# hanmekim/SceneLib2

Measured on NVIDIA H100. Metric: EKF-SLAM frames/sec @320x240 N=100 feats, higher is better.
Workload: dtype f64 (EKF, scores) + u8/int32 (correlation sums)

## Files before the change

### scenelib2_b200/csrc/search.cu

```cuda
#include "sl2_common.cuh"
#include "sl2_ptx.cuh"
#include "sl2_score.cuh"

namespace {

__device__ __forceinline__ void tma_load_3d(uint32_t dst, const CUtensorMap *map, uint32_t bar,
                                            int c0, int c1, int c2) {
  asm volatile(
      "cp.async.bulk.tensor.3d.shared::cluster.global.mbarrier::complete_tx::bytes "
      "[%0], [%1, {%3, %4, %5}], [%2];" ::"r"(dst),
      "l"(map), "r"(bar), "r"(c0), "r"(c1), "r"(c2)
      : "memory");
}

struct SearchLayout {
  int tcw, tch;
  int list, bar, vtab, per_warp;
};
__host__ __device__ inline SearchLayout search_layout(int tile_w, int tile_h, int box) {
  SearchLayout l;
  l.tcw = tile_w - 15 - box + 1;
  l.tch = tile_h - box + 1;
  const int tile_bytes = ((tile_w * tile_h + 16 + 127) / 128) * 128;
  const int max_tasks = l.tcw * ((l.tch + SL2_STRIP - 1) / SL2_STRIP);
  const int list_bytes = ((max_tasks * 4 + 15) / 16) * 16;
  const int col_bytes = ((l.tcw * 4 + 15) / 16) * 16;
  const int vtab_bytes = l.tch * 16 > col_bytes ? l.tch * 16 : col_bytes;
  l.list = tile_bytes;
  l.bar = tile_bytes + list_bytes;
  l.vtab = l.bar + 16;
  l.per_warp = ((l.vtab + vtab_bytes + 127) / 128) * 128;
  return l;
}

struct DumpPtrs {
  double *corr;
  double *sd;
  uint8_t *inside;
  int *box;
  int cap;
};

template <int BOX, bool FILTER>
__global__ void __launch_bounds__(SL2_SEARCH_WARPS * 32, FILTER ? (BOX <= 11 ? 4 : 3) : 2)
    search_kernel(const __grid_constant__ CUtensorMap tmap, const Sl2Dev d, const SearchLaunch L,
                  const DumpPtrs dump) {
  constexpr int NW = (BOX + 3) / 4;
  constexpr int HALF = (BOX - 1) / 2;
  constexpr int V = SL2_STRIP;
  constexpr uint32_t LASTMASK = (BOX % 4 == 0) ? 0xffffffffu : ((1u << (8 * (BOX % 4))) - 1u);
  extern __shared__ __align__(128) uint8_t smem[];
  pdl_prologue();

  const int warp = threadIdx.x >> 5, lane = threadIdx.x & 31;
  const int groups = (L.jobs_per_stream + SL2_SEARCH_WARPS - 1) / SL2_SEARCH_WARPS;
  const int sl = blockIdx.x / groups;
  const int r = (blockIdx.x % groups) * SL2_SEARCH_WARPS + warp;
  if (r >= L.jobs_per_stream) return;
  const int job = sl * L.jobs_per_stream + r;
  const int feat = L.job_feat[job];
  if (feat < 0) return;
  const int s = L.stream_lo + sl;

  const int TW = d.tile_w, TH = d.tile_h;
  const SearchLayout lay = search_layout(TW, TH, BOX);
  const int TCW = lay.tcw, TCH = lay.tch;
  uint8_t *tile = smem + (size_t)warp * lay.per_warp;
  uint32_t *list = reinterpret_cast<uint32_t *>(tile + lay.list);
  const uint32_t bar = smem_u32(tile + lay.bar);
  double2 *vtab = reinterpret_cast<double2 *>(tile + lay.vtab);
  short2 *colrange = reinterpret_cast<short2 *>(vtab);
  const uint32_t tile_s = smem_u32(tile);

  if (lane == 0) {
    mbar_init(bar, 1);
    fence_barrier_init();
    fence_proxy_async();
  }
  __syncwarp();

  uint32_t T[BOX][NW];
  {
    const uint32_t *pp =
        reinterpret_cast<const uint32_t *>(d.patches + ((size_t)s * d.Nmax + feat) * (BOX * 16));
#pragma unroll
    for (int rr = 0; rr < BOX; ++rr)
#pragma unroll
      for (int k = 0; k < NW; ++k) T[rr][k] = __ldg(pp + rr * 4 + k);
  }
  int Sg0 = 0, Sg0sq = 0;
#pragma unroll
  for (int rr = 0; rr < BOX; ++rr)
#pragma unroll
    for (int k = 0; k < NW; ++k) {
      Sg0 = __dp4a(T[rr][k], 0x01010101u, (uint32_t)Sg0);
      Sg0sq = __dp4a(T[rr][k], T[rr][k], (uint32_t)Sg0sq);
    }
  const PatchConst pconst = patch_const(BOX, Sg0, Sg0sq);
  const double V0d = fma(pconst.n, (double)Sg0sq, -((double)Sg0 * (double)Sg0));
  const float V0f = (float)V0d;
  const bool patch_ok = !(pconst.sigmag0 < 10.0);
  float bmin = 3.0e38f;

  const double P00 = L.job_puinv[job * 3 + 0], P01 = L.job_puinv[job * 3 + 1],
               P11 = L.job_puinv[job * 3 + 2];
  const double cx = L.job_centre[job * 2 + 0], cy = L.job_centre[job * 2 + 1];
  const int uc = __double2int_rz(add_(cx, 0.5));
  const int vc = __double2int_rz(add_(cy, 0.5));
  const SearchBox sb = search_box(P00, P01, P11, uc, vc, stream_width(d.cams[s]), stream_height(d.cams[s]), HALF);
  const Ellipse ell = make_ellipse(P00, P01, P11);
  const int CW = sb.cols(), CH = sb.rows();
  const int x0 = uc + sb.us - HALF, y0 = vc + sb.vs - HALF;
  if (!FILTER && lane == 0) {
    dump.box[0] = sb.us; dump.box[1] = sb.uf; dump.box[2] = sb.vs; dump.box[3] = sb.vf;
    dump.box[4] = uc; dump.box[5] = vc;
  }

  ScanBest best;
  uint32_t phase = 0;
  const int img = L.slot * d.B + s;

  if (CW > 0 && CH > 0) {
    for (int ty0 = 0; ty0 < CH; ty0 += TCH) {
      for (int tx0 = 0; tx0 < CW; tx0 += TCW) {
        const int tcw = min(TCW, CW - tx0), tch = min(TCH, CH - ty0);
        const int xa = (x0 + tx0) & ~15, xoff = (x0 + tx0) & 15;
        if (lane == 0) {
          mbar_expect_tx(bar, (uint32_t)(TW * TH));
          tma_load_3d(tile_s, &tmap, bar, xa, y0 + ty0, img);
        }
        const int nstrips = (tch + V - 1) / V;
        const int ntask = tcw * nstrips;
        int nlist = 0;
        if constexpr (FILTER) {
          const int vbase = sb.vs + ty0;
          for (int cu = lane; cu < tcw; cu += 32) {
            const Ellipse::Col col = ell.col((double)(sb.us + tx0 + cu));
            auto inside = [&](int cv) { return ell.inside(col, (double)(vbase + cv)); };
            int lo, hi;
            bool scan = !(P11 > 1e-7) || !(P11 < 1e7);
            if (!scan) {
              const double vx = -col.b / (2.0 * P11);
              const double disc = col.b * col.b - 4.0 * P11 * (col.a - 9.0);
              const float r = disc > 0.0 ? __fsqrt_rn((float)disc) / (float)(2.0 * P11) : 0.0f;
              const float lo_f = fminf(fmaxf(ceilf((float)vx - r) - (float)vbase, -1.0f), (float)tch);
              const float hi_f = fminf(fmaxf(floorf((float)vx + r) - (float)vbase, -1.0f), (float)tch);
              lo = max(0, min(tch - 1, (int)lo_f));
              hi = max(0, min(tch - 1, (int)hi_f));
              if (hi < lo) hi = lo;
              int it = 0;
              while (lo > 0 && it < 16 && inside(lo - 1)) { --lo; ++it; }
              while (lo <= hi && it < 16 && !inside(lo)) { ++lo; ++it; }
              if (it >= 16) {
                scan = true;
              } else if (lo > hi) {
                const int v0 = max(0, min(tch - 1, __float2int_rn((float)vx) - vbase));
                const int c0 = max(0, v0 - 1), c1 = min(tch - 1, v0 + 1);
                for (int cv = c0; cv <= c1; ++cv)
                  if (inside(cv)) scan = true;
              } else {
                while (hi < tch - 1 && it < 16 && inside(hi + 1)) { ++hi; ++it; }
                while (hi > lo && it < 16 && !inside(hi)) { --hi; ++it; }
                if (it >= 16) scan = true;
              }
            }
            if (scan) {
              lo = tch;
              hi = -1;
              for (int cv = 0; cv < tch; ++cv)
                if (inside(cv)) {
                  lo = min(lo, cv);
                  hi = cv;
                }
            }
            colrange[cu] = make_short2((short)lo, (short)hi);
          }
          __syncwarp();
          for (int sk = 0; sk < nstrips; ++sk) {
            const int st = (sk & 1) ? (nstrips - 1) / 2 + (sk + 1) / 2 : (nstrips - 1) / 2 - sk / 2;
            for (int cu0 = 0; cu0 < tcw; cu0 += 32) {
              const int cu = cu0 + lane;
              uint32_t entry = 0;
              if (cu < tcw) {
                const short2 rg = colrange[cu];
                const int jlo = max((int)rg.x - st * V, 0), jhi = min(min((int)rg.y - st * V, V - 1), tch - 1 - st * V);
                if (jlo <= jhi) {
                  const uint32_t mask = ((1u << (jhi + 1)) - 1u) & ~((1u << jlo) - 1u);
                  entry = (uint32_t)cu | ((uint32_t)st << 8) | (mask << 16);
                }
              }
              const uint32_t bal = __ballot_sync(0xffffffffu, entry != 0);
              if (entry) list[nlist + __popc(bal & ((1u << lane) - 1u))] = entry;
              nlist += __popc(bal);
            }
          }
        } else {
        for (int cv = lane; cv < tch; cv += 32) {
          const double dv = (double)(sb.vs + ty0 + cv);
          vtab[cv] = make_double2(dv, ell.vterm(dv));
        }
        __syncwarp();
        for (int t0 = 0; t0 < ntask; t0 += 32) {
          const int t = t0 + lane;
          uint32_t entry = 0;
          if (t < ntask) {
            const int sk = t / tcw, cu = t - sk * tcw;
            const int st = (sk & 1) ? (nstrips - 1) / 2 + (sk + 1) / 2 : (nstrips - 1) / 2 - sk / 2;
            const Ellipse::Col col = ell.col((double)(sb.us + tx0 + cu));
            uint32_t mask = 0;
#pragma unroll
            for (int j = 0; j < V; ++j) {
              const int cv = st * V + j;
              if (cv < tch) {
                const double2 tv = vtab[cv];
                mask |= (ell.inside(col, tv.x, tv.y) ? 1u : 0x100u) << j;
              }
            }
            if (mask) entry = (uint32_t)cu | ((uint32_t)st << 8) | (mask << 16);
          }
          const uint32_t bal = __ballot_sync(0xffffffffu, entry != 0);
          if (entry) list[nlist + __popc(bal & ((1u << lane) - 1u))] = entry;
          nlist += __popc(bal);
        }
        }
        __syncwarp();
        mbar_wait(bar, phase);
        phase ^= 1;

        for (int l0 = 0; l0 < nlist; l0 += 32) {
          const bool has_task = l0 + lane < nlist;
          uint32_t ax[V], a1[V], a2[V];
          float cap[V];
          int cand0 = 0;
#pragma unroll
          for (int j = 0; j < V; ++j) {
            ax[j] = a1[j] = a2[j] = 0;
            cap[j] = __int_as_float(0x7f800000);
          }
          if (has_task) {
            const uint32_t e = list[l0 + lane];
            const int cu = e & 0xff, st = (e >> 8) & 0xff;
            const uint32_t m_in = (e >> 16) & 0xff, m_all = m_in | ((e >> 24) & 0xff);
            const int cv0 = st * V;
            cand0 = (tx0 + cu) * CH + (ty0 + cv0);
            const int cx = cu + xoff;
            const int sh = (cx & 3) * 8;
            const uint32_t *wbase = reinterpret_cast<const uint32_t *>(tile) + (cx >> 2);
            const int tw4 = TW >> 2;
#pragma unroll
            for (int rr = 0; rr < V + BOX - 1; ++rr) {
              const int row = min(cv0 + rr, TH - 1);
              const uint32_t *wp = wbase + row * tw4;
              uint32_t w[NW + 1], sw[NW];
#pragma unroll
              for (int k = 0; k <= NW; ++k) w[k] = wp[k];
#pragma unroll
              for (int k = 0; k < NW; ++k) sw[k] = __funnelshift_r(w[k], w[k + 1], sh);
              sw[NW - 1] &= LASTMASK;
              uint32_t rs = 0, rq = 0;
#pragma unroll
              for (int k = 0; k < NW; ++k) {
                rs = __dp4a(sw[k], 0x01010101u, rs);
                rq = __dp4a(sw[k], sw[k], rq);
              }
#pragma unroll
              for (int j = 0; j < V; ++j) {
                const int t = rr - j;
                if (t >= 0 && t < BOX) {
#pragma unroll
                  for (int k = 0; k < NW; ++k) ax[j] = __dp4a(sw[k], T[t][k], ax[j]);
                  a1[j] += rs;
                  a2[j] += rq;
                }
              }
            }
            if constexpr (FILTER) {
              if (patch_ok) {
                float lmin = bmin;
#pragma unroll
                for (int j = 0; j < V; ++j) {
                  if ((m_in >> j) & 1u) {
                    if constexpr (BOX <= 11) {
                      constexpr uint32_t NN = BOX * BOX, T100u = 100u * NN * NN;
                      const uint32_t V1u = NN * a2[j] - a1[j] * a1[j];
                      if (V1u > T100u) {
                        const int N01i = (int)NN * (int)ax[j] - Sg0 * (int)a1[j];
                        const float rho = (float)N01i * rsqrtf(V0f * (float)V1u);
                        cap[j] = fmaf(-2.0f, rho, 2.0f);
                        lmin = fminf(lmin, cap[j]);
                      } else if (V1u == T100u) {
                        cap[j] = -3.0e38f;
                      }
                    } else {
                      constexpr uint32_t NN = BOX * BOX, T100u = 100u * NN * NN;
                      const uint32_t V1u = NN * a2[j] - a1[j] * a1[j];
                      if (V1u > T100u) {
                        const long long N01 = (long long)NN * (long long)ax[j] - (long long)Sg0 * (long long)a1[j];
                        const float rho = (float)N01 * rsqrtf(V0f * (float)V1u);
                        cap[j] = fmaf(-2.0f, rho, 2.0f);
                        lmin = fminf(lmin, cap[j]);
                      } else if (V1u == T100u) {
                        cap[j] = -3.0e38f;
                      }
                    }
                  }
                }
                bmin = lmin;
              }
            } else {
#pragma unroll
              for (int j = 0; j < V; ++j) {
                if ((m_all >> j) & 1u) {
                  const double Sg1d = (double)(int)a1[j], Sg1sqd = (double)(int)a2[j],
                               Sg0g1d = (double)(int)ax[j];
                  double sigmag1;
                  const double corr = exact_score_fn(pconst, Sg1d, Sg1sqd, Sg0g1d, &sigmag1);
                  const int ui = tx0 + cu, vi = ty0 + cv0 + j;
                  const int idx = ui * CH + vi;
                  const bool inside = (m_in >> j) & 1u;
                  if (idx < dump.cap) {
                    dump.corr[idx] = corr;
                    dump.sd[idx] = sigmag1;
                    dump.inside[idx] = inside ? 1 : 0;
                  }
                  if (inside && patch_ok && !(sigmag1 < 10.0)) best.offer(corr, idx);
                }
              }
            }
          }
          if constexpr (FILTER) {
#pragma unroll
            for (int o = 16; o > 0; o >>= 1) bmin = fminf(bmin, __shfl_xor_sync(0xffffffffu, bmin, o));
            const float thr = bmin + 1.0e-5f;
#pragma unroll
            for (int j = 0; j < V; ++j) {
              if (cap[j] <= thr) {
                double sg1;
                const double corr = exact_score_fn(pconst, (double)(int)a1[j], (double)(int)a2[j],
                                                   (double)(int)ax[j], &sg1);
                if (!(sg1 < 10.0)) best.offer(corr, cand0 + j);
              }
            }
          }
        }
        __syncwarp();
        fence_proxy_async();
      }
    }
  }

  best.warp_reduce();
  if (lane == 0) {
    const int2 uv = best.idx >= 0 ? scan_position(best.idx, CH, uc + sb.us, vc + sb.vs) : make_int2(-1, -1);
    const int u = uv.x, v = uv.y;
    const uint8_t ok = best.found();
    if (L.out_uv) {
      L.out_uv[job * 2 + 0] = u;
      L.out_uv[job * 2 + 1] = v;
    }
    if (L.out_found) L.out_found[job] = ok;
    if (L.out_best) L.out_best[job] = best.corr;
    if (L.scatter_to_features) {
      const size_t f = (size_t)s * d.Nmax + feat;
      d.z_uv[f * 2 + 0] = u;
      d.z_uv[f * 2 + 1] = v;
      d.found[f] = ok;
      d.best[f] = best.corr;
    }
  }
}

size_t search_smem_bytes(const Sl2Dev &d) {
  return (size_t)SL2_SEARCH_WARPS * search_layout(d.tile_w, d.tile_h, d.box).per_warp;
}

template <bool FILTER>
cudaError_t launch(const Sl2Dev &d, const CUtensorMap &tmap, const SearchLaunch &L, const DumpPtrs &dump,
                   Sl2Queue q) {
  return sl2_with_box(d.box, [&](auto box) {
    const int groups = (L.jobs_per_stream + SL2_SEARCH_WARPS - 1) / SL2_SEARCH_WARPS;
    const int grid = groups * L.stream_cnt;
    if (grid <= 0) return cudaSuccess;
    return sl2_launch_kernel(search_kernel<decltype(box)::value, FILTER>, dim3(grid), dim3(SL2_SEARCH_WARPS * 32),
                             search_smem_bytes(d), q, sl2_use_pdl(L.stream_cnt), tmap, d, L, dump);
  });
}

}

cudaError_t sl2_configure_search(const Sl2Dev &d) {
  const int smem = (int)search_smem_bytes(d);
  return sl2_with_box(d.box, [&](auto box) {
    constexpr int BOX = decltype(box)::value;
    cudaError_t e = cudaFuncSetAttribute(search_kernel<BOX, true>, cudaFuncAttributeMaxDynamicSharedMemorySize, smem);
    if (e == cudaSuccess)
      e = cudaFuncSetAttribute(search_kernel<BOX, false>, cudaFuncAttributeMaxDynamicSharedMemorySize, smem);
    return e;
  });
}

cudaError_t sl2_launch_search(const Sl2Dev &d, const CUtensorMap &tmap, const SearchLaunch &L, Sl2Queue q) {
  return launch<true>(d, tmap, L, DumpPtrs{}, q);
}

cudaError_t sl2_launch_score_map(const Sl2Dev &d, const CUtensorMap &tmap, int stream_id, int slot,
                                 const double *centre_dev, const double *puinv_dev, const int *feat_dev, int *box_dev,
                                 double *corr_dev, double *sd_dev, uint8_t *inside_dev, int cap, Sl2Queue q) {
  SearchLaunch L = {};
  L.job_centre = centre_dev;
  L.job_puinv = puinv_dev;
  L.job_feat = feat_dev;
  L.jobs_per_stream = 1;
  L.stream_lo = stream_id;
  L.stream_cnt = 1;
  L.slot = slot;
  const DumpPtrs dump = {corr_dev, sd_dev, inside_dev, box_dev, cap};
  return launch<false>(d, tmap, L, dump, q);
}
```

Measured before the change: 226,400.

## Restructure filtered patch search with longer strips, prefix sums and lazy exact rescoring

In the filtered search path, the strip length grows to 8 or 16 candidates, and window sums now come from running prefix sums instead of per-candidate accumulators. Exact double-precision scoring of the surviving candidates recomputes their correlation sums from shared memory rather than holding them in registers. The first TMA tile load is issued before the patch template is loaded, so the two overlap, and a division is replaced by a reciprocal multiply. The aim is lower register pressure and less redundant arithmetic per candidate. The risks are the recompute cost for survivors, the larger unrolled body, and a task list sized for the old strip length.

Result: faster. 233,700 (median of 6 runs) (+3.2%).

```diff
diff --git a/scenelib2_b200/csrc/search.cu b/scenelib2_b200/csrc/search.cu
--- a/scenelib2_b200/csrc/search.cu
+++ b/scenelib2_b200/csrc/search.cu
@@ -41,14 +41,44 @@
   int cap;
 };
 
+template <int BOX>
+__device__ __forceinline__ void window_row(const uint32_t *wp, int sh, uint32_t (&sw)[(BOX + 3) / 4]) {
+  constexpr int NW = (BOX + 3) / 4;
+  constexpr uint32_t LASTMASK = (BOX % 4 == 0) ? 0xffffffffu : ((1u << (8 * (BOX % 4))) - 1u);
+  uint32_t w[NW + 1];
+#pragma unroll
+  for (int k = 0; k <= NW; ++k) w[k] = wp[k];
+#pragma unroll
+  for (int k = 0; k < NW; ++k) sw[k] = __funnelshift_r(w[k], w[k + 1], sh);
+  sw[NW - 1] &= LASTMASK;
+}
+
+template <int BOX>
+__device__ __forceinline__ float approx_score(uint32_t ax, uint32_t a1, uint32_t a2, int Sg0, float V0f) {
+  constexpr uint32_t NN = BOX * BOX, T100u = 100u * NN * NN;
+  const uint32_t V1u = NN * a2 - a1 * a1;
+  if (V1u > T100u) {
+    float num;
+    if constexpr (BOX <= 11) {
+      num = (float)((int)NN * (int)ax - Sg0 * (int)a1);
+    } else {
+      num = (float)((long long)NN * (long long)ax - (long long)Sg0 * (long long)a1);
+    }
+    const float rho = num * rsqrtf(V0f * (float)V1u);
+    return fmaf(-2.0f, rho, 2.0f);
+  }
+  return V1u == T100u ? -3.0e38f : __int_as_float(0x7f800000);
+}
+
+__host__ __device__ constexpr int filter_strip(int box) { return box <= 11 ? 8 : 16; }
+
 template <int BOX, bool FILTER>
 __global__ void __launch_bounds__(SL2_SEARCH_WARPS * 32, FILTER ? (BOX <= 11 ? 4 : 3) : 2)
     search_kernel(const __grid_constant__ CUtensorMap tmap, const Sl2Dev d, const SearchLaunch L,
                   const DumpPtrs dump) {
   constexpr int NW = (BOX + 3) / 4;
   constexpr int HALF = (BOX - 1) / 2;
-  constexpr int V = SL2_STRIP;
-  constexpr uint32_t LASTMASK = (BOX % 4 == 0) ? 0xffffffffu : ((1u << (8 * (BOX % 4))) - 1u);
+  constexpr int V = FILTER ? filter_strip(BOX) : SL2_STRIP;
   extern __shared__ __align__(128) uint8_t smem[];
   pdl_prologue();
 
@@ -59,6 +89,9 @@
   if (r >= L.jobs_per_stream) return;
   const int job = sl * L.jobs_per_stream + r;
   const int feat = L.job_feat[job];
+  const double P00 = L.job_puinv[job * 3 + 0], P01 = L.job_puinv[job * 3 + 1],
+               P11 = L.job_puinv[job * 3 + 2];
+  const double cx = L.job_centre[job * 2 + 0], cy = L.job_centre[job * 2 + 1];
   if (feat < 0) return;
   const int s = L.stream_lo + sl;
 
@@ -79,32 +112,6 @@
   }
   __syncwarp();
 
-  uint32_t T[BOX][NW];
-  {
-    const uint32_t *pp =
-        reinterpret_cast<const uint32_t *>(d.patches + ((size_t)s * d.Nmax + feat) * (BOX * 16));
-#pragma unroll
-    for (int rr = 0; rr < BOX; ++rr)
-#pragma unroll
-      for (int k = 0; k < NW; ++k) T[rr][k] = __ldg(pp + rr * 4 + k);
-  }
-  int Sg0 = 0, Sg0sq = 0;
-#pragma unroll
-  for (int rr = 0; rr < BOX; ++rr)
-#pragma unroll
-    for (int k = 0; k < NW; ++k) {
-      Sg0 = __dp4a(T[rr][k], 0x01010101u, (uint32_t)Sg0);
-      Sg0sq = __dp4a(T[rr][k], T[rr][k], (uint32_t)Sg0sq);
-    }
-  const PatchConst pconst = patch_const(BOX, Sg0, Sg0sq);
-  const double V0d = fma(pconst.n, (double)Sg0sq, -((double)Sg0 * (double)Sg0));
-  const float V0f = (float)V0d;
-  const bool patch_ok = !(pconst.sigmag0 < 10.0);
-  float bmin = 3.0e38f;
-
-  const double P00 = L.job_puinv[job * 3 + 0], P01 = L.job_puinv[job * 3 + 1],
-               P11 = L.job_puinv[job * 3 + 2];
-  const double cx = L.job_centre[job * 2 + 0], cy = L.job_centre[job * 2 + 1];
   const int uc = __double2int_rz(add_(cx, 0.5));
   const int vc = __double2int_rz(add_(cy, 0.5));
   const SearchBox sb = search_box(P00, P01, P11, uc, vc, stream_width(d.cams[s]), stream_height(d.cams[s]), HALF);
@@ -116,33 +123,63 @@
     dump.box[4] = uc; dump.box[5] = vc;
   }
 
+  const int img = L.slot * d.B + s;
+  const auto stage = [&](int tx0, int ty0) {
+    if (lane == 0) {
+      mbar_expect_tx(bar, (uint32_t)(TW * TH));
+      tma_load_3d(tile_s, &tmap, bar, (x0 + tx0) & ~15, y0 + ty0, img);
+    }
+  };
+  if (CW > 0 && CH > 0) stage(0, 0);
+
+  uint32_t T[BOX][NW];
+  {
+    const uint32_t *pp =
+        reinterpret_cast<const uint32_t *>(d.patches + ((size_t)s * d.Nmax + feat) * (BOX * 16));
+#pragma unroll
+    for (int rr = 0; rr < BOX; ++rr)
+#pragma unroll
+      for (int k = 0; k < NW; ++k) T[rr][k] = __ldg(pp + rr * 4 + k);
+  }
+  int Sg0 = 0, Sg0sq = 0;
+#pragma unroll
+  for (int rr = 0; rr < BOX; ++rr)
+#pragma unroll
+    for (int k = 0; k < NW; ++k) {
+      Sg0 = __dp4a(T[rr][k], 0x01010101u, (uint32_t)Sg0);
+      Sg0sq = __dp4a(T[rr][k], T[rr][k], (uint32_t)Sg0sq);
+    }
+  const PatchConst pconst = patch_const(BOX, Sg0, Sg0sq);
+  const double V0d = fma(pconst.n, (double)Sg0sq, -((double)Sg0 * (double)Sg0));
+  const float V0f = (float)V0d;
+  const bool patch_ok = !(pconst.sigmag0 < 10.0);
+  float bmin = 3.0e38f;
+
   ScanBest best;
   uint32_t phase = 0;
-  const int img = L.slot * d.B + s;
 
   if (CW > 0 && CH > 0) {
     for (int ty0 = 0; ty0 < CH; ty0 += TCH) {
       for (int tx0 = 0; tx0 < CW; tx0 += TCW) {
         const int tcw = min(TCW, CW - tx0), tch = min(TCH, CH - ty0);
-        const int xa = (x0 + tx0) & ~15, xoff = (x0 + tx0) & 15;
-        if (lane == 0) {
-          mbar_expect_tx(bar, (uint32_t)(TW * TH));
-          tma_load_3d(tile_s, &tmap, bar, xa, y0 + ty0, img);
-        }
+        const int xoff = (x0 + tx0) & 15;
+        if (tx0 != 0 || ty0 != 0) stage(tx0, ty0);
         const int nstrips = (tch + V - 1) / V;
         const int ntask = tcw * nstrips;
         int nlist = 0;
         if constexpr (FILTER) {
           const int vbase = sb.vs + ty0;
+          const double r2p11 = 1.0 / (2.0 * P11);
+          const float r2p11f = (float)r2p11;
           for (int cu = lane; cu < tcw; cu += 32) {
             const Ellipse::Col col = ell.col((double)(sb.us + tx0 + cu));
             auto inside = [&](int cv) { return ell.inside(col, (double)(vbase + cv)); };
             int lo, hi;
             bool scan = !(P11 > 1e-7) || !(P11 < 1e7);
             if (!scan) {
-              const double vx = -col.b / (2.0 * P11);
+              const double vx = -col.b * r2p11;
               const double disc = col.b * col.b - 4.0 * P11 * (col.a - 9.0);
-              const float r = disc > 0.0 ? __fsqrt_rn((float)disc) / (float)(2.0 * P11) : 0.0f;
+              const float r = disc > 0.0 ? __fsqrt_rn((float)disc) * r2p11f : 0.0f;
               const float lo_f = fminf(fmaxf(ceilf((float)vx - r) - (float)vbase, -1.0f), (float)tch);
               const float hi_f = fminf(fmaxf(floorf((float)vx + r) - (float)vbase, -1.0f), (float)tch);
               lo = max(0, min(tch - 1, (int)lo_f));
@@ -227,36 +264,102 @@
         mbar_wait(bar, phase);
         phase ^= 1;
 
-        for (int l0 = 0; l0 < nlist; l0 += 32) {
-          const bool has_task = l0 + lane < nlist;
-          uint32_t ax[V], a1[V], a2[V];
-          float cap[V];
-          int cand0 = 0;
-#pragma unroll
-          for (int j = 0; j < V; ++j) {
-            ax[j] = a1[j] = a2[j] = 0;
-            cap[j] = __int_as_float(0x7f800000);
+        const int tw4 = TW >> 2;
+        if constexpr (FILTER) {
+          static_assert(V <= 16, "the task entry holds a 16-bit candidate mask");
+          static_assert(V >= SL2_STRIP, "the task list is sized for strips of SL2_STRIP candidates");
+          for (int l0 = 0; l0 < nlist; l0 += 32) {
+            float cap[V];
+#pragma unroll
+            for (int j = 0; j < V; ++j) cap[j] = __int_as_float(0x7f800000);
+            int cv0 = 0, cand0 = 0;
+            int sh = 0;
+            const uint32_t *wbase = nullptr;
+            if (l0 + lane < nlist && patch_ok) {
+              const uint32_t e = list[l0 + lane];
+              const int cu = e & 0xff, st = (e >> 8) & 0xff;
+              const uint32_t m_in = e >> 16;
+              cv0 = st * V;
+              cand0 = (tx0 + cu) * CH + (ty0 + cv0);
+              const int cx = cu + xoff;
+              sh = (cx & 3) * 8;
+              wbase = reinterpret_cast<const uint32_t *>(tile) + (cx >> 2);
+              uint32_t ax[V], h1[V], h2[V], s1 = 0, s2 = 0;
+              float lmin = bmin;
+#pragma unroll
+              for (int j = 0; j < V; ++j) ax[j] = 0;
+#pragma unroll
+              for (int rr = 0; rr < V + BOX - 1; ++rr) {
+                uint32_t sw[NW];
+                window_row<BOX>(wbase + min(cv0 + rr, TH - 1) * tw4, sh, sw);
+                if (rr < V) {
+                  h1[rr] = s1;
+                  h2[rr] = s2;
+                }
+#pragma unroll
+                for (int k = 0; k < NW; ++k) {
+                  s1 = __dp4a(sw[k], 0x01010101u, s1);
+                  s2 = __dp4a(sw[k], sw[k], s2);
+                }
+#pragma unroll
+                for (int j = 0; j < V; ++j) {
+                  const int t = rr - j;
+                  if (t >= 0 && t < BOX) {
+#pragma unroll
+                    for (int k = 0; k < NW; ++k) ax[j] = __dp4a(sw[k], T[t][k], ax[j]);
+                  }
+                }
+                const int j = rr - (BOX - 1);
+                if (j >= 0 && ((m_in >> j) & 1u)) {
+                  cap[j] = approx_score<BOX>(ax[j], s1 - h1[j], s2 - h2[j], Sg0, V0f);
+                  if (cap[j] > -1.0e38f) lmin = fminf(lmin, cap[j]);
+                }
+              }
+              bmin = lmin;
+            }
+#pragma unroll
+            for (int o = 16; o > 0; o >>= 1) bmin = fminf(bmin, __shfl_xor_sync(0xffffffffu, bmin, o));
+            const float thr = bmin + 1.0e-5f;
+            uint32_t surv = 0;
+#pragma unroll
+            for (int j = 0; j < V; ++j) surv |= (cap[j] <= thr ? 1u : 0u) << j;
+            while (surv) {
+              const int j = __ffs(surv) - 1;
+              surv &= surv - 1;
+              uint32_t ax = 0, a1 = 0, a2 = 0;
+#pragma unroll
+              for (int t = 0; t < BOX; ++t) {
+                uint32_t sw[NW];
+                window_row<BOX>(wbase + (cv0 + j + t) * tw4, sh, sw);
+#pragma unroll
+                for (int k = 0; k < NW; ++k) {
+                  ax = __dp4a(sw[k], T[t][k], ax);
+                  a1 = __dp4a(sw[k], 0x01010101u, a1);
+                  a2 = __dp4a(sw[k], sw[k], a2);
+                }
+              }
+              double sg1;
+              const double corr = exact_score_fn(pconst, (double)(int)a1, (double)(int)a2, (double)(int)ax, &sg1);
+              if (!(sg1 < 10.0)) best.offer(corr, cand0 + j);
+            }
           }
-          if (has_task) {
+        } else {
+          for (int l0 = 0; l0 < nlist; l0 += 32) {
+            if (l0 + lane >= nlist) continue;
+            uint32_t ax[V], a1[V], a2[V];
+#pragma unroll
+            for (int j = 0; j < V; ++j) ax[j] = a1[j] = a2[j] = 0;
             const uint32_t e = list[l0 + lane];
             const int cu = e & 0xff, st = (e >> 8) & 0xff;
             const uint32_t m_in = (e >> 16) & 0xff, m_all = m_in | ((e >> 24) & 0xff);
             const int cv0 = st * V;
-            cand0 = (tx0 + cu) * CH + (ty0 + cv0);
             const int cx = cu + xoff;
             const int sh = (cx & 3) * 8;
             const uint32_t *wbase = reinterpret_cast<const uint32_t *>(tile) + (cx >> 2);
-            const int tw4 = TW >> 2;
 #pragma unroll
             for (int rr = 0; rr < V + BOX - 1; ++rr) {
-              const int row = min(cv0 + rr, TH - 1);
-              const uint32_t *wp = wbase + row * tw4;
-              uint32_t w[NW + 1], sw[NW];
-#pragma unroll
-              for (int k = 0; k <= NW; ++k) w[k] = wp[k];
-#pragma unroll
-              for (int k = 0; k < NW; ++k) sw[k] = __funnelshift_r(w[k], w[k + 1], sh);
-              sw[NW - 1] &= LASTMASK;
+              uint32_t sw[NW];
+              window_row<BOX>(wbase + min(cv0 + rr, TH - 1) * tw4, sh, sw);
               uint32_t rs = 0, rq = 0;
 #pragma unroll
               for (int k = 0; k < NW; ++k) {
@@ -274,71 +377,22 @@
                 }
               }
             }
-            if constexpr (FILTER) {
-              if (patch_ok) {
-                float lmin = bmin;
-#pragma unroll
-                for (int j = 0; j < V; ++j) {
-                  if ((m_in >> j) & 1u) {
-                    if constexpr (BOX <= 11) {
-                      constexpr uint32_t NN = BOX * BOX, T100u = 100u * NN * NN;
-                      const uint32_t V1u = NN * a2[j] - a1[j] * a1[j];
-                      if (V1u > T100u) {
-                        const int N01i = (int)NN * (int)ax[j] - Sg0 * (int)a1[j];
-                        const float rho = (float)N01i * rsqrtf(V0f * (float)V1u);
-                        cap[j] = fmaf(-2.0f, rho, 2.0f);
-                        lmin = fminf(lmin, cap[j]);
-                      } else if (V1u == T100u) {
-                        cap[j] = -3.0e38f;
-                      }
-                    } else {
-                      constexpr uint32_t NN = BOX * BOX, T100u = 100u * NN * NN;
-                      const uint32_t V1u = NN * a2[j] - a1[j] * a1[j];
-                      if (V1u > T100u) {
-                        const long long N01 = (long long)NN * (long long)ax[j] - (long long)Sg0 * (long long)a1[j];
-                        const float rho = (float)N01 * rsqrtf(V0f * (float)V1u);
-                        cap[j] = fmaf(-2.0f, rho, 2.0f);
-                        lmin = fminf(lmin, cap[j]);
-                      } else if (V1u == T100u) {
-                        cap[j] = -3.0e38f;
-                      }
-                    }
-                  }
-                }
-                bmin = lmin;
-              }
-            } else {
-#pragma unroll
-              for (int j = 0; j < V; ++j) {
-                if ((m_all >> j) & 1u) {
-                  const double Sg1d = (double)(int)a1[j], Sg1sqd = (double)(int)a2[j],
-                               Sg0g1d = (double)(int)ax[j];
-                  double sigmag1;
-                  const double corr = exact_score_fn(pconst, Sg1d, Sg1sqd, Sg0g1d, &sigmag1);
-                  const int ui = tx0 + cu, vi = ty0 + cv0 + j;
-                  const int idx = ui * CH + vi;
-                  const bool inside = (m_in >> j) & 1u;
-                  if (idx < dump.cap) {
-                    dump.corr[idx] = corr;
-                    dump.sd[idx] = sigmag1;
-                    dump.inside[idx] = inside ? 1 : 0;
-                  }
-                  if (inside && patch_ok && !(sigmag1 < 10.0)) best.offer(corr, idx);
-                }
-              }
-            }
-          }
-          if constexpr (FILTER) {
-#pragma unroll
-            for (int o = 16; o > 0; o >>= 1) bmin = fminf(bmin, __shfl_xor_sync(0xffffffffu, bmin, o));
-            const float thr = bmin + 1.0e-5f;
 #pragma unroll
             for (int j = 0; j < V; ++j) {
-              if (cap[j] <= thr) {
-                double sg1;
-                const double corr = exact_score_fn(pconst, (double)(int)a1[j], (double)(int)a2[j],
-                                                   (double)(int)ax[j], &sg1);
-                if (!(sg1 < 10.0)) best.offer(corr, cand0 + j);
+              if ((m_all >> j) & 1u) {
+                const double Sg1d = (double)(int)a1[j], Sg1sqd = (double)(int)a2[j],
+                             Sg0g1d = (double)(int)ax[j];
+                double sigmag1;
+                const double corr = exact_score_fn(pconst, Sg1d, Sg1sqd, Sg0g1d, &sigmag1);
+                const int ui = tx0 + cu, vi = ty0 + cv0 + j;
+                const int idx = ui * CH + vi;
+                const bool inside = (m_in >> j) & 1u;
+                if (idx < dump.cap) {
+                  dump.corr[idx] = corr;
+                  dump.sd[idx] = sigmag1;
+                  dump.inside[idx] = inside ? 1 : 0;
+                }
+                if (inside && patch_ok && !(sigmag1 < 10.0)) best.offer(corr, idx);
               }
             }
           }
```
